# SarodYatawatta/federated-pytorch-test

Measured on NVIDIA H100. Metric: train_images_per_sec, higher is better.
Workload: dtype tf32

## Files before the change

federated_pytorch_test_b200/csrc/bindings.cpp:

```cpp
#include <ATen/cuda/CUDAContext.h>
#include <c10/cuda/CUDAGuard.h>
#include <torch/extension.h>

#include <cstdlib>

#include "fedb200.h"

namespace fb = fedb200;
using torch::Tensor;

static cudaStream_t cur_stream() { return at::cuda::getCurrentCUDAStream().stream(); }
static const float* fptr(const Tensor& t) { return t.data_ptr<float>(); }
static float* fptr_mut(Tensor& t) { return t.data_ptr<float>(); }
static const float* opt_ptr(const c10::optional<Tensor>& t) { return (t.has_value() && t->defined()) ? t->data_ptr<float>() : nullptr; }

#define CHECK_F32_CUDA(x) TORCH_CHECK((x).is_cuda() && (x).scalar_type() == torch::kFloat32, #x " must be a CUDA float32 tensor")
#define CHECK_CONTIG(x) TORCH_CHECK((x).is_contiguous(), #x " must be contiguous")

void adam_prox(Tensor x, Tensor g, Tensor m, Tensor v, Tensor step, double lr, double b1, double b2, double eps,
               c10::optional<Tensor> z, c10::optional<Tensor> y, double rho, double l1, double l2,
               c10::optional<Tensor> rho_dev) {
  CHECK_F32_CUDA(x); CHECK_CONTIG(x); CHECK_CONTIG(g); CHECK_CONTIG(m); CHECK_CONTIG(v);
  c10::cuda::CUDAGuard guard(x.device());
  fb::adam_prox(fptr_mut(x), fptr(g), fptr_mut(m), fptr_mut(v), step.data_ptr<int>(), (int)x.numel(), (float)lr, (float)b1,
// ... 262 lines not shown
  return out;
}

Tensor linear_tf32(Tensor x, Tensor w, c10::optional<Tensor> bias, bool act) {
  CHECK_F32_CUDA(x); CHECK_F32_CUDA(w); CHECK_CONTIG(x); CHECK_CONTIG(w);
  TORCH_CHECK(x.dim() == 2 && w.dim() == 2 && x.size(1) == w.size(1), "linear_tf32: x [M,K], w [N,K]");
  c10::cuda::CUDAGuard guard(x.device());
  const int M = (int)x.size(0), K = (int)x.size(1), N = (int)w.size(0);
  auto out = torch::empty({M, N}, x.options());
  fb::linear_tf32(fptr(x), fptr(w), opt_ptr(bias), fptr_mut(out), M, N, K, K, K, N, act ? 1 : 0, cur_stream());
  return out;
}
bool conv_supported(int64_t H_out, int64_t W_out, int64_t C_in, int64_t stride) {
  return fb::conv_geometry_supported((int)H_out, (int)W_out, (int)C_in, (int)stride);
}
int64_t conv_orientation(int64_t NB, int64_t H_out, int64_t W_out, int64_t C_out, int64_t stride) {
  return fb::pick_conv_orientation((int)NB, (int)H_out, (int)W_out, (int)C_out, (int)stride);
}
bool conv_window_reuse(int64_t H_out, int64_t W_out, int64_t C_in, int64_t C_out, int64_t kh, int64_t stride, int64_t dil) {
  return fb::conv_window_reuse((int)H_out, (int)W_out, (int)C_in, (int)C_out, (int)kh, (int)stride, (int)dil);
}
Tensor conv2d_nhwc(Tensor x, Tensor w, c10::optional<Tensor> stats, int64_t stride, int64_t pad, int64_t dil, int64_t orient) {
  CHECK_F32_CUDA(x); CHECK_F32_CUDA(w); CHECK_CONTIG(x); CHECK_CONTIG(w);
  TORCH_CHECK(x.dim() == 4 && w.dim() == 4 && x.size(3) == w.size(3), "conv2d_nhwc: x [N,H,W,Ci], w [Co,kh,kw,Ci]");
  c10::cuda::CUDAGuard guard(x.device());
  const int NB = (int)x.size(0), H = (int)x.size(1), W = (int)x.size(2), Ci = (int)x.size(3);
  const int Co = (int)w.size(0), kh = (int)w.size(1), kw = (int)w.size(2);
  const int Ho = (H + 2 * (int)pad - (int)dil * (kh - 1) - 1) / (int)stride + 1;
  const int Wo = (W + 2 * (int)pad - (int)dil * (kw - 1) - 1) / (int)stride + 1;
  auto y = torch::empty({NB, Ho, Wo, Co}, x.options());
  float* st = (stats.has_value() && stats->defined()) ? stats->data_ptr<float>() : nullptr;
  fb::conv2d_nhwc_tf32(fptr(x), fptr(w), fptr_mut(y), st, NB, H, W, Ci, Co, kh, kw, (int)stride, (int)pad, (int)dil, Ho, Wo, cur_stream(),
                       (int)orient);
  return y;
}

Tensor conv2d_nhwc_sized(Tensor x, Tensor w, c10::optional<Tensor> stats, int64_t stride, int64_t pad, int64_t dil,
                         int64_t Ho, int64_t Wo) {
  CHECK_F32_CUDA(x); CHECK_F32_CUDA(w); CHECK_CONTIG(x); CHECK_CONTIG(w);
  TORCH_CHECK(x.dim() == 4 && w.dim() == 4 && x.size(3) == w.size(3), "conv2d_nhwc: x [N,H,W,Ci], w [Co,kh,kw,Ci]");
  TORCH_CHECK(Ho > 0 && Wo > 0, "conv2d_nhwc_sized: positive output size");
  c10::cuda::CUDAGuard guard(x.device());
  const int NB = (int)x.size(0), H = (int)x.size(1), W = (int)x.size(2), Ci = (int)x.size(3);
  const int Co = (int)w.size(0), kh = (int)w.size(1), kw = (int)w.size(2);
  auto y = torch::empty({NB, Ho, Wo, Co}, x.options());
  float* st = (stats.has_value() && stats->defined()) ? stats->data_ptr<float>() : nullptr;
  fb::conv2d_nhwc_tf32(fptr(x), fptr(w), fptr_mut(y), st, NB, H, W, Ci, Co, kh, kw, (int)stride, (int)pad, (int)dil, (int)Ho,
                       (int)Wo, cur_stream());
  return y;
}

bool conv_wgrad_supported(int64_t Cx, int64_t Co, int64_t stride, int64_t Wo, int64_t Ho) {
  return fb::conv_wgrad_supported((int)Cx, (int)Co, (int)stride, (int)Wo, (int)Ho);
}
void conv_wgrad(Tensor x, Tensor dy, Tensor dw, int64_t stride, int64_t pad, int64_t dil) {
  CHECK_F32_CUDA(x); CHECK_F32_CUDA(dy); CHECK_F32_CUDA(dw); CHECK_CONTIG(x); CHECK_CONTIG(dy); CHECK_CONTIG(dw);
  TORCH_CHECK(x.dim() == 4 && dy.dim() == 4 && dw.dim() == 4 && x.size(0) == dy.size(0) && dw.size(0) == dy.size(3) &&
              dw.size(3) <= x.size(3), "conv_wgrad: x [N,H,W,Cx], dy [N,Ho,Wo,Co], dw [Co,kh,kw,Cw<=Cx]");
  c10::cuda::CUDAGuard guard(x.device());
  const int NB = (int)x.size(0), H = (int)x.size(1), W = (int)x.size(2), Cx = (int)x.size(3);
  const int Ho = (int)dy.size(1), Wo = (int)dy.size(2), Co = (int)dy.size(3);
  const int kh = (int)dw.size(1), kw = (int)dw.size(2), Cw = (int)dw.size(3);
  fb::conv_wgrad_tf32(fptr(x), fptr(dy), fptr_mut(dw), NB, H, W, Cx, Cw, Co, kh, kw, (int)stride, (int)pad, (int)dil, Ho, Wo,
                      cur_stream());
}

// ... 534 lines not shown
  m.def("l1_l2", &l1_l2);
  m.def("make_pair", &make_pair);
  m.def("welford", &welford);
  m.def("penalty_value", &penalty_value);
  m.def("penalty_grad", &penalty_grad);
  m.def("multi_dot", &multi_dot);
  m.def("lbfgs_two_loop", &lbfgs_two_loop);
  m.def("normalize_u8", &normalize_u8);
  m.def("augment_normalize_u8", &augment_normalize_u8, py::arg("u8"), py::arg("rows"), py::arg("key"), py::arg("counter"),
        py::arg("mean"), py::arg("std"), py::arg("to_nchw"));
  m.def("col_stats", &col_stats);
  m.def("head_fwd", &head_fwd);
  m.def("head_bwd", &head_bwd);
  m.def("bn_elu_fwd", &bn_elu_fwd, py::arg("y"), py::arg("stats"), py::arg("gamma"), py::arg("beta"), py::arg("residual"),
        py::arg("running_mean"), py::arg("running_var"), py::arg("eps"), py::arg("momentum"), py::arg("act"),
        py::arg("self_clean"), py::arg("use_running") = false);
  m.def("bn_elu_bwd", &bn_elu_bwd);
  m.def("gn_elu_fwd", &gn_elu_fwd, py::arg("y"), py::arg("gamma"), py::arg("beta"), py::arg("residual"), py::arg("groups"),
        py::arg("eps"), py::arg("act"));
  m.def("gn_elu_bwd", &gn_elu_bwd, py::arg("dout"), py::arg("out"), py::arg("y"), py::arg("mean"), py::arg("rstd"),
        py::arg("gamma"), py::arg("beta"), py::arg("groups"), py::arg("want_dres"), py::arg("act"), py::arg("want_affine"));
  m.def("avgpool_nhwc", &avgpool_nhwc);
  m.def("avgpool_nhwc_bwd", &avgpool_nhwc_bwd);
  m.def("weight_flip", &weight_flip);
  m.def("convT_pack", &convT_pack);
  m.def("linear_tf32", &linear_tf32);
  m.def("conv_supported", &conv_supported);
  m.def("conv_orientation", &conv_orientation);
  m.def("conv_window_reuse", &conv_window_reuse, py::arg("H_out"), py::arg("W_out"), py::arg("C_in"), py::arg("C_out"), py::arg("kh"),
        py::arg("stride") = 1, py::arg("dil") = 1);
  m.def("conv2d_nhwc", &conv2d_nhwc, py::arg("x"), py::arg("w"), py::arg("stats"), py::arg("stride"), py::arg("pad"), py::arg("dil"),
        py::arg("orient") = -1);
  m.def("conv2d_nhwc_sized", &conv2d_nhwc_sized);
  m.def("conv2d_nhwc_bias_act", &conv2d_nhwc_bias_act);
  m.def("conv2d_nhwc_bn_eval", &conv2d_nhwc_bn_eval);
  m.def("conv2d_nhwc_shuffle", &conv2d_nhwc_shuffle);
  m.def("conv_shuffle_supported", &conv_shuffle_supported);
  m.def("conv2d_nhwc_multidil", &conv2d_nhwc_multidil);
  m.def("conv_multidil_supported", &conv_multidil_supported);
  m.def("conv_wgrad", &conv_wgrad);
  m.def("conv_wgrad_supported", &conv_wgrad_supported);
  m.def("cross_entropy_fwd", &cross_entropy_fwd);
  m.def("cross_entropy_bwd", &cross_entropy_bwd);
  m.def("vae_loss_fwd", &vae_loss_fwd);
  m.def("vae_loss_bwd", &vae_loss_bwd);
  m.def("linear_f32", &linear_f32);
  m.def("linear_f32_dgrad", &linear_f32_dgrad);
  m.def("linear_f32_wgrad", &linear_f32_wgrad);
  m.def("act_bwd_bias", &act_bwd_bias);
  m.def("maxpool2x2_fwd", &maxpool2x2_fwd);
  m.def("maxpool2x2_bwd", &maxpool2x2_bwd);
  m.def("argmax_count", &argmax_count);
  m.def("info_nce_max_p", &info_nce_max_p);
  m.def("info_nce_scratch_floats", &info_nce_scratch_floats);
  m.def("info_nce_fwd", &info_nce_fwd);
  m.def("info_nce_bwd", &info_nce_bwd);
  m.def("gauss_nll_rows_fwd", &gauss_nll_rows_fwd);
  m.def("gauss_nll_rows_bwd", &gauss_nll_rows_bwd);
  m.def("smallconv_supported", &smallconv_supported);
  m.def("smallconv_fwd", &smallconv_fwd);
  m.def("smallconv_unpool_actbwd", &smallconv_unpool_actbwd);
  m.def("smallconv_dgrad", &smallconv_dgrad);
  m.def("smallconv_wgrad", &smallconv_wgrad);
  m.def("block_reduce", &block_reduce);
  m.def("block_reduce_fedopt", &block_reduce_fedopt);
  m.def("dp_clip", &dp_clip);
// ... 6 lines not shown
```

federated_pytorch_test_b200/csrc/fedb200.h:

```cpp
#pragma once
#include <cuda_runtime.h>
#include <stdint.h>

namespace fedb200 {

void count_launch(int n = 1);
long long launch_count();

bool pdl_enabled();
#ifdef __CUDACC__
__device__ __forceinline__ void pdl_wait() { asm volatile("griddepcontrol.wait;" ::: "memory"); }
__device__ __forceinline__ void pdl_launch_dependents() { asm volatile("griddepcontrol.launch_dependents;" ::: "memory"); }
__device__ __forceinline__ void pdl_prologue() {
  pdl_launch_dependents();
  pdl_wait();
}
template <typename... KArgs, typename... Args>
inline cudaError_t launch_pdl(void (*kernel)(KArgs...), dim3 grid, dim3 block, size_t smem, cudaStream_t stream,
                              Args&&... args) {
  cudaLaunchConfig_t cfg{};
  cfg.gridDim = grid;
  cfg.blockDim = block;
  cfg.dynamicSmemBytes = smem;
  cfg.stream = stream;
  cudaLaunchAttribute attr[1];
  attr[0].id = cudaLaunchAttributeProgrammaticStreamSerialization;
  attr[0].val.programmaticStreamSerializationAllowed = pdl_enabled() ? 1 : 0;
  cfg.attrs = attr;
  cfg.numAttrs = 1;
  return cudaLaunchKernelEx(&cfg, kernel, KArgs(args)...);
}
#endif

int pick_block_n(int M, int N);
void linear_tf32(const float* x, const float* w, const float* bias, float* out, int M, int N, int K, int ldx, int ldw,
                 int ldo, int act, cudaStream_t stream);
bool conv_geometry_supported(int H_out, int W_out, int C_in, int stride);
enum { CONV_ORIENT_AUTO = -1, CONV_ORIENT_ROW = 0, CONV_ORIENT_PIXEL = 1, CONV_ORIENT_PIXEL_PERTAP = 2 };
int pick_conv_orientation(int NB, int H_out, int W_out, int C_out, int stride);
bool conv_window_reuse(int H_out, int W_out, int C_in, int C_out, int kh, int stride, int dil);
void conv2d_nhwc_tf32(const float* x, const float* w, float* y, float* stats, int NB, int H, int W, int C_in, int C_out,
                      int kh, int kw, int stride, int pad, int dil, int H_out, int W_out, cudaStream_t stream,
                      int orient = CONV_ORIENT_AUTO);
void conv2d_nhwc_bias_act_tf32(const float* x, const float* w, const float* bias, int act, float* y, int NB, int H, int W,
                               int C_in, int C_out, int kh, int kw, int stride, int pad, int dil, int H_out, int W_out,
                               cudaStream_t stream);
void conv2d_nhwc_bn_eval_tf32(const float* x, const float* w, const float* gamma, const float* beta, const float* mean,
                              const float* var, float eps, const float* residual, int act, float* y, int NB, int H, int W,
                              int C_in, int C_out, int kh, int kw, int stride, int pad, int dil, int H_out, int W_out,
                              cudaStream_t stream);

bool conv_shuffle_supported(int H_out, int W_out, int C_in, int Ci_out);
void conv2d_nhwc_shuffle_tf32(const float* x, const float* w, float* out, int NB, int H, int W, int C_in, int C4, int kh, int kw,
                              int pad, int H_out, int W_out, cudaStream_t stream);
bool conv_multidil_supported(int H_out, int W_out, int C_in, int stride, int branches);
void conv2d_nhwc_multidil_tf32(const float* x, const float* w, const float* bias, int act, float* y, int NB, int H, int W, int C_in,
                               int C_out, int branches, int kh, int kw, int stride, const int* dils, const int* pads, int H_out,
                               int W_out, cudaStream_t stream);
bool conv_wgrad_supported(int C_x, int C_out, int stride, int W_out, int H_out);
void conv_wgrad_tf32(const float* x, const float* dy, float* dw, int NB, int H, int W, int C_x, int C_w, int C_out, int kh,
                     int kw, int stride, int pad, int dil, int H_out, int W_out, cudaStream_t stream);


void adam_prox(float* x, const float* g, float* m, float* v, const int* step_dev, int n, float lr, float b1, float b2,
               float eps, const float* z, const float* y, float rho, float l1, float l2, cudaStream_t s,
               const float* rho_dev = nullptr);
void sgd_prox(float* x, const float* g, float* buf, int n, float lr, float momentum, bool nesterov, float weight_decay,
              const float* z, const float* y, float rho, float l1, float l2, cudaStream_t s, const float* rho_dev);
void bump_step(int* step_dev, cudaStream_t s);
void l1_l2(const float* g, int n, float* out2, cudaStream_t s);
void make_pair(const float* g, const float* gprev, const float* d, float t, float trust, float* y, float* sv, int n,
               float* out3, cudaStream_t s);
void welford(const float* g, float* mean, float* m2, int n, float inv_n, float* out1, cudaStream_t s);
void penalty_value(const float* x, const float* z, const float* y, float rho, float l1, float l2, int n, float* out1,
                   cudaStream_t s);
void penalty_grad(float* g, const float* x, const float* z, const float* y, float rho, float l1, float l2, int n,
// ... 193 lines not shown
```

federated_pytorch_test_b200/csrc/gemm_wgmma.cu:

```cuda
#include "fedb200.h"
#include "igemm_wgmma.cuh"
#include "wgrad_wgmma.cuh"

#include <algorithm>
#include <cstdlib>
#include <mutex>
#include <stdexcept>
#include <string>

namespace fedb200 {

typedef CUresult (*EncodeTiledFn)(CUtensorMap*, CUtensorMapDataType, cuuint32_t, void*, const cuuint64_t*,
                                  const cuuint64_t*, const cuuint32_t*, const cuuint32_t*, CUtensorMapInterleave,
                                  CUtensorMapSwizzle, CUtensorMapL2promotion, CUtensorMapFloatOOBfill);

static EncodeTiledFn encode_fn() {
  static EncodeTiledFn fn = nullptr;
  static std::once_flag once;
  std::call_once(once, [] {
    void* p = nullptr;
    cudaDriverEntryPointQueryResult q;
    cudaError_t e = cudaGetDriverEntryPoint("cuTensorMapEncodeTiled", &p, cudaEnableDefault, &q);
    if (e != cudaSuccess || q != cudaDriverEntryPointSuccess || p == nullptr)
      throw std::runtime_error("fedb200: cuTensorMapEncodeTiled unavailable (no CUDA driver?)");
// ... 187 lines not shown

static int pix_window_stage_bytes(int H_out, int W_out, int C_in, int C_out, int kh, int stride, int dil) {
  if (C_out != 64 || stride != 1 || dil != 1 || kh != PIX_WIN_KH || C_in % IG_BLOCK_K != 0) return 0;
  if (!pix_geometry_supported(H_out, W_out, 1) || PX_BLOCK_M / W_out > H_out || (W_out * IG_BLOCK_K * 4) % 1024 != 0) return 0;
  const int win_rows = PX_BLOCK_M / W_out + kh - 1;
  if (win_rows > 256) return 0;
  const int stage = (win_rows * W_out + kh * C_out) * IG_BLOCK_K * 4;
  return PixSmem<64, PIX_WIN_STAGES>::window_total(stage) <= 227 * 1024 ? stage : 0;
}

bool conv_window_reuse(int H_out, int W_out, int C_in, int C_out, int kh, int stride, int dil) {
  return pix_window_stage_bytes(H_out, W_out, C_in, C_out, kh, stride, dil) > 0;
}

int pick_conv_orientation(int NB, int H_out, int W_out, int C_out, int stride) {
  if (env_int("FEDB200_BLOCK_N", 0) != 0) return CONV_ORIENT_ROW;
  if (C_out != 64 && C_out != 128) return CONV_ORIENT_ROW;
  if (!pix_geometry_supported(H_out, W_out, stride)) return CONV_ORIENT_ROW;
  const long long tiles = (static_cast<long long>(NB) * H_out * W_out + PX_BLOCK_M - 1) / PX_BLOCK_M;
  return tiles >= num_sms() - num_sms() / 8 ? CONV_ORIENT_PIXEL : CONV_ORIENT_ROW;
}

struct BnEvalArgs {
  const float* gamma;
  const float* beta;
  const float* mean;
  const float* var;
  float eps;
  const float* residual;
};

static void conv2d_generic(const float* x, const float* w, float* y, float* stats, const float* bias, int act, int NB, int H,
                           int W, int C_in, int C_out, int kh, int kw, int stride, int pad, int dil, int H_out, int W_out,
                           cudaStream_t stream, const BnEvalArgs* eval_bn = nullptr, int orient = CONV_ORIENT_ROW);

void conv2d_nhwc_tf32(const float* x, const float* w, float* y, float* stats, int NB, int H, int W, int C_in, int C_out,
                      int kh, int kw, int stride, int pad, int dil, int H_out, int W_out, cudaStream_t stream, int orient) {
  if (orient == CONV_ORIENT_AUTO) orient = pick_conv_orientation(NB, H_out, W_out, C_out, stride);
  conv2d_generic(x, w, y, stats, nullptr, 0, NB, H, W, C_in, C_out, kh, kw, stride, pad, dil, H_out, W_out, stream, nullptr,
                 orient);
}

void conv2d_nhwc_bias_act_tf32(const float* x, const float* w, const float* bias, int act, float* y, int NB, int H, int W,
                               int C_in, int C_out, int kh, int kw, int stride, int pad, int dil, int H_out, int W_out,
                               cudaStream_t stream) {
  conv2d_generic(x, w, y, nullptr, bias, act, NB, H, W, C_in, C_out, kh, kw, stride, pad, dil, H_out, W_out, stream);
}

void conv2d_nhwc_bn_eval_tf32(const float* x, const float* w, const float* gamma, const float* beta, const float* mean,
                              const float* var, float eps, const float* residual, int act, float* y, int NB, int H, int W,
                              int C_in, int C_out, int kh, int kw, int stride, int pad, int dil, int H_out, int W_out,
                              cudaStream_t stream) {
  const BnEvalArgs args{gamma, beta, mean, var, eps, residual};
  conv2d_generic(x, w, y, nullptr, nullptr, act, NB, H, W, C_in, C_out, kh, kw, stride, pad, dil, H_out, W_out, stream, &args);
}

static int pick_tap_pack(int C_in) {
  if (env_int("FEDB200_TAP_PACK", 1) == 0 || C_in > 16 || (C_in & 3)) return IG_BLOCK_K;
  return C_in <= 8 ? 8 : 16;
}

static void conv2d_generic(const float* x, const float* w, float* y, float* stats, const float* bias, int act, int NB, int H,
                           int W, int C_in, int C_out, int kh, int kw, int stride, int pad, int dil, int H_out, int W_out,
                           cudaStream_t stream, const BnEvalArgs* eval_bn, int orient) {
  if (!conv_geometry_supported(H_out, W_out, C_in, stride))
    throw std::runtime_error("fedb200: conv geometry not supported by the wgmma path");
  const bool pix = orient == CONV_ORIENT_PIXEL || orient == CONV_ORIENT_PIXEL_PERTAP;
  if (pix && ((C_out != 64 && C_out != 128) || bias != nullptr || act != 0 || eval_bn != nullptr ||
              !pix_geometry_supported(H_out, W_out, stride) || (reinterpret_cast<uintptr_t>(y) & 15) != 0))
    throw std::runtime_error("fedb200: pixel-major convolution needs C_out 64 / 128, a plain or statistics epilogue, "
                             "whole-row 256-pixel tiles and a 16-byte aligned output");
  const int win_stage = orient == CONV_ORIENT_PIXEL ? pix_window_stage_bytes(H_out, W_out, C_in, C_out, kh, stride, dil) : 0;
  const int tile_m = pix ? PX_BLOCK_M : IG_BLOCK_M;
  const int rows = tile_m / W_out;
  const int boxH = rows <= H_out ? rows : H_out;
  const int boxN = rows <= H_out ? 1 : rows / H_out;
  const int M = NB * H_out * W_out;
  const int bn = pix ? C_out : pick_block_n(M, C_out);
  const int cw = pick_tap_pack(C_in);
  CUtensorMap ta = make_tmap_nhwc(x, NB, H, W, C_in, boxN, win_stage ? boxH + kh - 1 : boxH, W_out, stride, cw);
  CUtensorMap tb = make_tmap_2d(w, C_out, uint64_t(kh) * kw * C_in, uint64_t(kh) * kw * C_in, bn, cw);
  IgemmParams p{};
  p.M = M; p.N = C_out;
  p.cblocks = (C_in + IG_BLOCK_K - 1) / IG_BLOCK_K;
  p.num_k_blocks = kh * kw * p.cblocks;
  p.taps_total = kh * kw;
  if (cw != IG_BLOCK_K) {
    p.cw = cw;
    p.num_k_blocks = (kh * kw + IG_BLOCK_K / cw - 1) / (IG_BLOCK_K / cw);
  }
  p.taps_w = kw; p.b_cols_per_tap = C_in; p.is_conv = 1;
  p.HW_out = H_out * W_out; p.W_out = W_out;
  p.stride = stride; p.pad = pad; p.dil = dil;
  p.out = y; p.ldo = C_out; p.bias = bias; p.act = act; p.stats = stats;
  p.k_splits = 1; p.kb_per_split = p.num_k_blocks;
  if (win_stage) {
    p.num_k_blocks = kw * p.cblocks;
    p.kb_per_split = p.num_k_blocks;
    p.win_rows = boxH + kh - 1;
    p.win_a_bytes = p.win_rows * W_out * IG_BLOCK_K * 4;
    p.win_stage_bytes = win_stage;
    launch_pix<64, PIX_WIN_KH>(ta, tb, p, stream);
    return;
  }
  if (pix) {
    if (C_out == 64) launch_pix<64, 0>(ta, tb, p, stream);
    else launch_pix<128, 0>(ta, tb, p, stream);
    return;
  }
  if (bias == nullptr && (act == 0 || eval_bn != nullptr)) {
    const int splits = pick_k_splits(M, C_out, bn, p.num_k_blocks);
    if (splits > 1) {
      p.kb_per_split = (p.num_k_blocks + splits - 1) / splits;
      p.k_splits = (p.num_k_blocks + p.kb_per_split - 1) / p.kb_per_split;
      p.stats = nullptr;
      cudaMemsetAsync(y, 0, size_t(M) * C_out * sizeof(float), stream);
    }
  }
  if (eval_bn != nullptr) {
    if ((C_out & 3) != 0) throw std::runtime_error("fedb200: eval-mode BatchNorm epilogue needs C_out % 4 == 0");
    if (p.k_splits > 1) {
      p.act = 0;
    } else {
      p.bn_gamma = eval_bn->gamma; p.bn_beta = eval_bn->beta; p.bn_mean = eval_bn->mean; p.bn_var = eval_bn->var;
      p.bn_eps = eval_bn->eps; p.residual = eval_bn->residual; p.ldr = C_out;
    }
  }
  dispatch(bn, ta, tb, p, stream);
  if (p.k_splits > 1 && stats != nullptr) col_stats(y, stats, M, C_out, stream);
  if (p.k_splits > 1 && eval_bn != nullptr)
    bn_elu_fwd(y, nullptr, eval_bn->gamma, eval_bn->beta, eval_bn->residual, y, const_cast<float*>(eval_bn->mean),
               const_cast<float*>(eval_bn->var), nullptr, nullptr, M, C_out, eval_bn->eps, 0.f, act, 0, stream, 1);
}

bool conv_shuffle_supported(int H_out, int W_out, int C_in, int Ci_out) {
  if (!conv_geometry_supported(H_out, W_out, C_in, 1)) return false;
  if (Ci_out % 32 != 0) return false;
  if (W_out > 32 || (32 % W_out) != 0) return false;
  return true;
}

void conv2d_nhwc_shuffle_tf32(const float* x, const float* w, float* out, int NB, int H, int W, int C_in, int C4, int kh, int kw,
                              int pad, int H_out, int W_out, cudaStream_t stream) {
  const int Ci = C4 / 4;
  if (!conv_shuffle_supported(H_out, W_out, C_in, Ci)) throw std::runtime_error("fedb200: shuffled conv store not supported for this shape");
  const int rows = 128 / W_out;
  const int boxH = rows <= H_out ? rows : H_out;
  const int boxN = rows <= H_out ? 1 : rows / H_out;
  const int M = NB * H_out * W_out;
// ... 134 lines not shown
```

federated_pytorch_test_b200/csrc/igemm_wgmma.cuh:

```cuda
#pragma once
#include "sm90.cuh"
#include "fedb200.h"

namespace fedb200 {

constexpr int IG_BLOCK_M = 128;
constexpr int IG_BLOCK_K = 32;
constexpr int IG_MMA_K = 8;
constexpr int IG_THREADS = 384;

struct IgemmParams {
  int M, N;
  int num_k_blocks;
  int cblocks;
  int taps_w;
  int b_cols_per_tap;
  int is_conv;
  int HW_out, W_out;
  int stride, pad, dil;
  float* out;
  int ldo;
  const float* bias;
  int act;
  float* stats;
  int kb_per_split;
  int k_splits;
  int m_tiles, n_tiles, total_tiles;
  int shuffle_ci;
  int tma_store;
  int cw;
  int taps_total;
  int ms_kh;
  unsigned long long ms_dil, ms_pad;
  const float* bn_gamma;
  const float* bn_beta;
  const float* bn_mean;
  const float* bn_var;
  float bn_eps;
  const float* residual;
  int ldr;
  int win_rows;
  int win_a_bytes;
  int win_stage_bytes;
};

template <int BLOCK_N, int STAGES>
struct IgemmSmem {
  static constexpr int A_BYTES = IG_BLOCK_M * IG_BLOCK_K * 4;
  static constexpr int B_BYTES = BLOCK_N * IG_BLOCK_K * 4;
  static constexpr int STAGE_BYTES = A_BYTES + B_BYTES;
  static constexpr int STAGING_BYTES = 2 * 64 * 32 * 4;
  static constexpr int STATS_BYTES = 8 * 2 * BLOCK_N * 4;
  static constexpr int BAR_BYTES = 2 * STAGES * 8;
  static constexpr int TOTAL = STAGES * STAGE_BYTES + STAGING_BYTES + STATS_BYTES + BAR_BYTES + 1024;
};

struct TileCoord {
  int m0, n0, kb_begin, kb_count;
};
__device__ __forceinline__ TileCoord decode_tile(const IgemmParams& p, int t, int block_m, int block_n) {
  const int n_idx = t % p.n_tiles;
  const int rest = t / p.n_tiles;
  const int m_idx = rest % p.m_tiles;
  const int z = rest / p.m_tiles;
  TileCoord c;
  c.m0 = m_idx * block_m;
  c.n0 = n_idx * block_n;
  c.kb_begin = z * p.kb_per_split;
  c.kb_count = min(p.kb_per_split, p.num_k_blocks - c.kb_begin);
  return c;
}

__device__ __forceinline__ void named_bar_sync(uint32_t id, uint32_t n) {
  asm volatile("bar.sync %0, %1;" ::"r"(id), "r"(n) : "memory");
}
__device__ __forceinline__ void named_bar_arrive(uint32_t id, uint32_t n) {
// ... 212 lines not shown
          }
        }
      }
    }
    if (p.tma_store) {
#pragma unroll
      for (int c0 = 0; c0 < BLOCK_N; c0 += 32) {
        if (tid == 0) tma_store_wait_read();
        named_bar_sync(wg_bar, 128);
#pragma unroll
        for (int ii = 0; ii < 4; ++ii) {
          const int i = c0 / 8 + ii;
          const int cc = 8 * ii + col_in;
#pragma unroll
          for (int h = 0; h < 2; ++h) {
            const int r = row_in + 8 * h;
            const int rr = r & 31;
            float* dst = stg + (r >> 5) * 1024 + rr * 32 + (((uint32_t(cc) >> 2) ^ uint32_t(rr & 7)) << 2) + (cc & 3);
            *reinterpret_cast<float2*>(dst) = make_float2(acc[4 * i + 2 * h], acc[4 * i + 2 * h + 1]);
          }
        }
        fence_proxy_async();
        named_bar_sync(wg_bar, 128);
        if (tid == 0) {
          const int pc = c.n0 + c0;
          for (int b = 0; b < 2; ++b) {
            const int row0 = c.m0 + 64 * g + 32 * b;
            if (row0 >= p.M || pc >= p.N) continue;
            const float* src = stg + b * 1024;
            if (p.shuffle_ci > 0) {
              const int phase = pc / p.shuffle_ci;
              if (p.k_splits > 1) tma_reduce_add_5d(&tmap_c, src, pc - phase * p.shuffle_ci, phase & 1, 0, phase >> 1, row0 / p.W_out);
              else tma_store_5d(&tmap_c, src, pc - phase * p.shuffle_ci, phase & 1, 0, phase >> 1, row0 / p.W_out);
            } else if (p.k_splits > 1) {
              tma_reduce_add_2d(&tmap_c, src, pc, row0);
            } else {
              tma_store_2d(&tmap_c, src, pc, row0);
            }
          }
          tma_store_commit();
        }
      }
    } else {
#pragma unroll
      for (int i = 0; i < NACC / 4; ++i) {
#pragma unroll
        for (int h = 0; h < 2; ++h) {
          const int row = h ? row_b : row_a;
          if (!(h ? ok_b : ok_a)) continue;
#pragma unroll
          for (int e = 0; e < 2; ++e) {
            const int col = c.n0 + 8 * i + col_in + e;
            if (col >= p.N) continue;
            float* dst = p.out + size_t(row) * p.ldo + col;
            if (p.k_splits > 1) atomicAdd(dst, acc[4 * i + 2 * h + e]);
            else *dst = acc[4 * i + 2 * h + e];
          }
        }
      }
    }
    if (p.stats != nullptr) {
      named_bar_sync(3, 256);
      for (int j = threadIdx.x - 128; j < 2 * BLOCK_N; j += 256) {
        float v = 0.f;
#pragma unroll
        for (int w = 0; w < 8; ++w) v += colsum[w * 2 * BLOCK_N + j];
        const int cc = j < BLOCK_N ? j : j - BLOCK_N;
        if (c.n0 + cc < p.N) atomicAdd(p.stats + (j < BLOCK_N ? 0 : p.N) + c.n0 + cc, v);
      }
      named_bar_sync(3, 256);
    }
  }
  if (p.tma_store && tid == 0) tma_store_wait_read();
}

constexpr int PX_BLOCK_M = 256;

template <int CO, int STAGES>
struct PixSmem {
  static constexpr int A_BYTES = PX_BLOCK_M * IG_BLOCK_K * 4;
  static constexpr int B_BYTES = CO * IG_BLOCK_K * 4;
  static constexpr int STAGE_BYTES = A_BYTES + B_BYTES;
  static constexpr int STAGING_BYTES = 2 * 2 * 2 * 32 * 32 * 4;
  static constexpr int BAR_BYTES = 2 * STAGES * 8;
  static constexpr int TOTAL = STAGES * STAGE_BYTES + STAGING_BYTES + BAR_BYTES + 1024;
  static constexpr int window_total(int stage_bytes) { return STAGES * stage_bytes + STAGING_BYTES + BAR_BYTES + 1024; }
};

// ... 158 lines not shown
      if ((lane & 3) == 0) {
        const int ca = ch_wg + ch_lo;
        atomicAdd(p.stats + ca, s1a);
        atomicAdd(p.stats + p.N + ca, s2a);
        atomicAdd(p.stats + ca + 8, s1b);
        atomicAdd(p.stats + p.N + ca + 8, s2b);
      }
    }
#pragma unroll
    for (int q = 0; q < PX_BLOCK_M / 32; ++q) {
      float* buf = stg + (q & 1) * 2048;
      if (tid == 0) tma_store_wait_read_n<1>();
      named_bar_sync(wg_bar, 128);
#pragma unroll
      for (int ii = 0; ii < 4; ++ii) {
        const int i = 4 * q + ii;
#pragma unroll
        for (int h = 0; h < 2; ++h) {
          const int ch = ch_lo + 8 * h;
          const int cc = ch & 31;
#pragma unroll
          for (int e = 0; e < 2; ++e) {
            const int px = 8 * ii + px_in + e;
            buf[(ch >> 5) * 1024 + px * 32 + (((uint32_t(cc) >> 2) ^ uint32_t(px & 7)) << 2) + (cc & 3)] = acc[4 * i + 2 * h + e];
          }
        }
      }
      fence_proxy_async();
      named_bar_sync(wg_bar, 128);
      if (tid == 0) {
        const int row0 = c.m0 + 32 * q;
        if (row0 < p.M) {
#pragma unroll
          for (int b = 0; b < 2; ++b) tma_store_2d(&tmap_c, buf + b * 1024, ch_wg + 32 * b, row0);
        }
        tma_store_commit();
      }
    }
  }
  if (tid == 0) tma_store_wait_read();
}

}
```

federated_pytorch_test_b200/models/resnet.py:

```python
from __future__ import annotations

import functools
from typing import Callable, List, Type

import torch
import torch.nn as nn
import torch.nn.functional as F

from .base import BlockPartitioned
from ..ops import functional as FX


def _conv3x3(cin: int, cout: int, stride: int) -> nn.Conv2d:
    return nn.Conv2d(cin, cout, kernel_size=3, stride=stride, padding=1, bias=False)


def _conv1x1(cin: int, cout: int, stride: int) -> nn.Conv2d:
    return nn.Conv2d(cin, cout, kernel_size=1, stride=stride, bias=False)


def norm_layer(norm: str = "batch", groups: int = 32) -> Callable[[int], nn.Module]:
    if norm == "batch":
        return nn.BatchNorm2d
    if norm == "group":
        return functools.partial(nn.GroupNorm, groups)
    raise ValueError("norm must be 'batch' or 'group', got %r" % (norm,))


class _Residual(nn.Module):

    expansion = 1

    def _make_shortcut(self, in_planes: int, out_planes: int, stride: int, norm) -> None:
        if stride != 1 or in_planes != out_planes:
            self.shortcut = nn.Sequential(_conv1x1(in_planes, out_planes, stride), norm(out_planes))
        else:
            self.shortcut = nn.Sequential()

    def _skip(self, x: torch.Tensor) -> torch.Tensor:
        if len(self.shortcut) == 0:
            return x
        return FX.conv_bn_act(x, self.shortcut[0], self.shortcut[1], act=False)


class BasicBlock(_Residual):
    expansion = 1

    def __init__(self, in_planes: int, planes: int, stride: int = 1, norm=nn.BatchNorm2d):
        super().__init__()
        self.conv1 = _conv3x3(in_planes, planes, stride)
        self.bn1 = norm(planes)
        self.conv2 = _conv3x3(planes, planes, 1)
        self.bn2 = norm(planes)
        self._make_shortcut(in_planes, planes * self.expansion, stride, norm)

    def forward(self, x: torch.Tensor) -> torch.Tensor:
        h = FX.conv_bn_act(x, self.conv1, self.bn1, act=True)
        return FX.conv_bn_act(h, self.conv2, self.bn2, residual=self._skip(x), act=True)


class Bottleneck(_Residual):
    expansion = 4

    def __init__(self, in_planes: int, planes: int, stride: int = 1, norm=nn.BatchNorm2d):
        super().__init__()
        self.conv1 = _conv1x1(in_planes, planes, 1)
        self.bn1 = norm(planes)
        self.conv2 = _conv3x3(planes, planes, stride)
        self.bn2 = norm(planes)
        self.conv3 = _conv1x1(planes, planes * self.expansion, 1)
        self.bn3 = norm(planes * self.expansion)
        self._make_shortcut(in_planes, planes * self.expansion, stride, norm)

    def forward(self, x: torch.Tensor) -> torch.Tensor:
        h = FX.conv_bn_act(x, self.conv1, self.bn1, act=True)
        h = FX.conv_bn_act(h, self.conv2, self.bn2, act=True)
        return FX.conv_bn_act(h, self.conv3, self.bn3, residual=self._skip(x), act=True)


class ResNet(BlockPartitioned):
    _TABLES = {
        18: ((0, 2), (3, 8), (9, 14), (15, 23), (24, 29), (30, 38), (39, 44), (45, 53), (54, 59), (60, 61)),
        9: ((0, 2), (3, 8), (9, 14), (15, 17), (18, 23), (24, 29), (30, 32), (33, 37)),
    }
    LINEAR_IDS = ()

    def __init__(self, block: Type[_Residual], num_blocks: List[int], qualifier: int, num_classes: int = 10,
                 norm: str = "batch", groups: int = 32):
        super().__init__()
# ... 36 lines not shown
```

federated_pytorch_test_b200/ops/cuda_ops.py:

```python
from __future__ import annotations

from typing import List, Optional, Sequence, Tuple

import torch
import torch.nn as nn
import torch.nn.functional as F

from .. import _ext
from . import conv_math

_EXT = None


def ext():
    global _EXT
    if _EXT is None:
        _EXT = _ext.load("fedb200_cuda", required=True)
    return _EXT


def launch_count() -> int:
    return int(ext().launch_count())


# ... 305 lines not shown
    def forward(ctx, x, weight, gamma, beta, residual, running_mean, running_var, stride, pad, eps, momentum, act):
        e = ext()
        xn = _nhwc(x)
        wk = _krsc(weight)
        if xn.shape[3] == 3:
            xn = F.pad(xn, (0, 1))
            wk = F.pad(wk, (0, 1))
        Co = weight.shape[0]
        stats, self_clean = _stats_buffer(weight, Co)
        y = e.conv2d_nhwc(xn, wk, stats, stride, pad, 1)
        res = _nhwc(residual) if residual is not None else None
        out, mean, invstd = e.bn_elu_fwd(y, stats, gamma, beta, res, running_mean, running_var, eps, momentum, act, self_clean)
        ctx.save_for_backward(xn, wk, y, out, mean, invstd, gamma, beta)
        ctx.cfg = (stride, pad, act, residual is not None, tuple(weight.shape), x.shape[1])
        ctx.w_persistent = _aliases(wk, weight)
        ctx.weight_ref = weight
        return out.permute(0, 3, 1, 2)

    @staticmethod
    def backward(ctx, dout):
        e = ext()
        xn, wk, y, out, mean, invstd, gamma, beta = ctx.saved_tensors
        stride, pad, act, has_res, wshape, cin_logical = ctx.cfg
        need_x, need_w, need_g, need_b, need_r = ctx.needs_input_grad[:5]
        dn = _nhwc(dout)
        dgamma = torch.zeros_like(gamma) if need_g else None
        dbeta = torch.zeros_like(gamma) if need_b else None
        dy, dres = e.bn_elu_bwd(dn, out if (has_res or not act) else None, y, mean, invstd, gamma, beta, dgamma, dbeta,
                                bool(has_res and need_r), act, _bwd_sums_buffer(gamma, gamma.numel()))
        dx, dw = _conv_backward(e, xn, wk, dy, stride, pad, wshape, cin_logical, need_x, need_w, ctx.w_persistent,
                                ctx.weight_ref)
        dr = dres.permute(0, 3, 1, 2) if (has_res and need_r and dres is not None) else None
        return dx, dw, dgamma, dbeta, dr, None, None, None, None, None, None, None


def _conv_backward(e, xn, wk, dy, stride, pad, wshape, cin_logical, need_x, need_w, w_persistent, weight_ref):
    dx = dw = None
    kh, kw = wshape[2], wshape[3]
    if need_x:
        Ci = xn.shape[3]
        if stride == 1 and e.conv_supported(xn.shape[1], xn.shape[2], wshape[0], 1) and Ci % 4 == 0:
            dxn = e.conv2d_nhwc(dy, _flipped_weight(wk, need_w, w_persistent), None, 1, kh - 1 - pad, 1)
        elif stride == 2 and _s2_dgrad_supported(e, xn, dy, kh, kw, pad):
            dxn = _s2_dgrad(e, dy, wk, need_w, w_persistent)
        else:
            dxn = torch.ops.aten.convolution_backward(
                dy.permute(0, 3, 1, 2), xn.permute(0, 3, 1, 2), wk.permute(0, 3, 1, 2), None,
                [stride, stride], [pad, pad], [1, 1], False, [0, 0], 1, [True, False, False])[0]
            dxn = _nhwc(dxn)
        if dxn.shape[3] != cin_logical:
            dxn = dxn[..., :cin_logical]
        dx = dxn.permute(0, 3, 1, 2)
    if need_w:
        if conv_wgrad_supported(xn, dy, stride):
            dw = conv_wgrad(xn, dy, kh, kw, cin_logical, stride, pad, 1, weight_ref)
        else:
            dwk = torch.ops.aten.convolution_backward(
                dy.permute(0, 3, 1, 2), xn.permute(0, 3, 1, 2), wk.permute(0, 3, 1, 2), None,
                [stride, stride], [pad, pad], [1, 1], False, [0, 0], 1, [False, True, False])[1]
            dw = dwk[:, :cin_logical] if dwk.shape[1] != cin_logical else dwk
    return dx, dw


def conv_gn_act_supported(x: torch.Tensor, conv: nn.Conv2d, gn: nn.GroupNorm) -> bool:
    if not isinstance(gn, nn.GroupNorm) or not gn.affine or gn.weight.dtype != torch.float32:
        return False
# ... 585 lines not shown
```

federated_pytorch_test_b200/ops/functional.py:

```python
from __future__ import annotations

import os
from typing import Optional

import torch
import torch.nn as nn
import torch.nn.functional as F

_FAST = {"enabled": os.environ.get("FEDB200_FAST", "1") != "0"}


def set_fast_path(flag: bool) -> None:
    _FAST["enabled"] = bool(flag)


def fast_path_enabled() -> bool:
    return _FAST["enabled"]


def _use_fast(x: torch.Tensor) -> bool:
    return _FAST["enabled"] and x.is_cuda


def conv_bn_act(
    x: torch.Tensor,
    conv: nn.Conv2d,
    bn: nn.BatchNorm2d,
    residual: Optional[torch.Tensor] = None,
    act: bool = True,
) -> torch.Tensor:
    if _use_fast(x):
        from . import cuda_ops

        if cuda_ops.conv_bn_act_eval_supported(x, conv, bn, residual):
            return cuda_ops.conv_bn_act_eval(x, conv, bn, residual, act)
        if cuda_ops.conv_bn_act_supported(x, conv, bn):
            return cuda_ops.conv_bn_act(x, conv, bn, residual, act)
        if cuda_ops.conv_gn_act_supported(x, conv, bn):
            return cuda_ops.conv_gn_act(x, conv, bn, residual, act)
    y = F.conv2d(x, conv.weight, conv.bias, conv.stride, conv.padding, conv.dilation, conv.groups)
    y = bn(y)
    if residual is not None:
        y = y + residual
    return F.elu(y) if act else y


def pool_linear(x: torch.Tensor, linear: nn.Linear, window: int = 4) -> torch.Tensor:
    if _use_fast(x):
        from . import cuda_ops

        if cuda_ops.pool_linear_supported(x, linear, window):
            return cuda_ops.pool_linear(x, linear, window)
    y = F.avg_pool2d(x, window)
    return F.linear(y.reshape(y.shape[0], -1), linear.weight, linear.bias)


def conv_act(x: torch.Tensor, conv: nn.Module, act: bool = True) -> torch.Tensor:
    if _use_fast(x):
        from . import cuda_ops

        if cuda_ops.conv_act_supported(x, conv) or cuda_ops.conv_transpose_act_supported(x, conv):
            return cuda_ops.conv_act(x, conv, act)
        if cuda_ops.conv1x1_supported(x, conv):
            return cuda_ops.conv1x1_linear(x, conv, act)
        if cuda_ops.unfold_conv_supported(x, conv):
            return cuda_ops.unfold_conv(x, conv, act)
        if cuda_ops.smallconv_supported(x, conv):
            return cuda_ops.small_conv(x, conv, act, False)
    y = conv(x)
    return F.elu(y) if act else y


def dilated_stem(x: torch.Tensor, convs, act: bool = True) -> torch.Tensor:
    if _use_fast(x):
        from . import cuda_ops

        if cuda_ops.dilated_stem_supported(x, convs):
# ... 43 lines not shown
```

Measured before the change: 36590.

## Fuse residual skip gradient into conv data-gradient via accumulating store

```diff
diff --git a/baseline/profile_step.py b/baseline/profile_step.py
--- /dev/null
+++ b/baseline/profile_step.py
@@ -0,0 +1,124 @@
+from __future__ import annotations
+
+import argparse
+import collections
+import json
+import os
+import subprocess
+import sys
+
+import torch
+
+ROOT = os.path.dirname(os.path.dirname(os.path.abspath(__file__)))
+if ROOT not in sys.path:
+    sys.path.insert(0, ROOT)
+
+STEPS_PER_ROUND = 49
+CATEGORIES = ("conv forward", "data gradient", "weight gradient", "bn_elu_fwd", "bn_elu_bwd reduce/apply",
+              "ATen elementwise", "head / loss / optimizer", "rest")
+
+
+def category(name: str, backward: bool) -> str:
+    if "igemm_wgmma" in name:
+        return "data gradient" if backward else "conv forward"
+    if "wgrad_wgmma" in name:
+        return "weight gradient"
+    if "bn_elu_fwd" in name:
+        return "bn_elu_fwd"
+    if "bn_elu_bwd" in name:
+        return "bn_elu_bwd reduce/apply"
+    if "at::native" in name or "elementwise" in name.lower():
+        return "ATen elementwise"
+    if any(k in name for k in ("head_", "ce_fwd", "ce_bwd", "adam_prox", "sgd_prox", "bump_step", "avgpool", "penalty")):
+        return "head / loss / optimizer"
+    return "rest"
+
+
+def device_info() -> str:
+    try:
+        q = subprocess.run(["nvidia-smi", "--query-gpu=name,power.limit,clocks.max.sm", "--format=csv,noheader"],
+                           capture_output=True, text=True, timeout=30).stdout.strip()
+    except (OSError, subprocess.SubprocessError):
+        q = ""
+    return q or torch.cuda.get_device_name()
+
+
+def main() -> None:
+    ap = argparse.ArgumentParser()
+    ap.add_argument("--warmup", type=int, default=8)
+    ap.add_argument("--steps", type=int, default=20)
+    args = ap.parse_args()
+    assert torch.cuda.is_available(), "profile_step.py measures on the GPU"
+    assert args.warmup + 2 * args.steps < STEPS_PER_ROUND, "both windows must lie inside the first round"
+
+    from federated_pytorch_test_b200.algo.engine import Engine
+    from federated_pytorch_test_b200.algo.strategies import FedAvg
+    from federated_pytorch_test_b200.api import common, federated_multi
+
+    cfg = federated_multi.Config(K=1, use_resnet=True, Nloop=1000, Nadmm=3, Nepoch=1, check_results=False, save_model=False,
+                                 be_verbose=False, biased_input=True, data_on_device=True, graphs=True, fast=True,
+                                 collective="auto", diagnostics="post", max_minibatches=STEPS_PER_ROUND, seed=69,
+                                 optimizer="adam")
+    topo, coll = common.setup_runtime(cfg)
+    task = common.ClassifierTask(cfg, topo, cfg.lambda1, cfg.lambda2)
+    eng = Engine(task, topo, FedAvg(coll, topo), coll, common.engine_config(cfg), log=lambda m: None)
+
+    p0, p1 = args.warmup, args.warmup + args.steps
+    t1 = p1 + args.steps
+    prof = torch.profiler.profile(activities=[torch.profiler.ProfilerActivity.CUDA])
+    ev = [torch.cuda.Event(enable_timing=True), torch.cuda.Event(enable_timing=True)]
+
+    def hook(e: Engine) -> None:
+        n = e.steps_done
+        if n == p0:
+            torch.cuda.synchronize()
+            prof.start()
+        elif n == p1:
+            torch.cuda.synchronize()
+            prof.stop()
+            ev[0].record()
+        elif n == t1:
+            ev[1].record()
+            torch.cuda.synchronize()
+            e.stop_requested = True
+
+    eng.step_hook = hook
+    eng.run()
+    step_ms = ev[0].elapsed_time(ev[1]) / args.steps
+
+    kernels = sorted((k for k in prof.events() if k.device_type == torch.autograd.DeviceType.CUDA and k.device_time > 0),
+                     key=lambda k: k.time_range.start)
+    per_name = collections.defaultdict(float)
+    launches = collections.Counter()
+    backward = False
+    for k in kernels:
+        name = k.name
+        if "ce_bwd" in name or "head_bwd" in name:
+            backward = True
+        cat = category(name, backward)
+        if "adam_prox" in name or "sgd_prox" in name:
+            backward = False
+        short = name.split("(")[0].replace("void ", "").replace("fedb200::", "")
+        per_name[(cat, short)] += k.device_time / 1e3 / args.steps
+        launches[(cat, short)] += 1
+    per_cat = collections.defaultdict(float)
+    for (cat, _), t in per_name.items():
+        per_cat[cat] += t
+    total = sum(per_cat.values())
+
+    print("device:", device_info())
+    print("%-28s %10s %8s" % ("category / kernel", "us/step", "launches"))
+    for cat in CATEGORIES:
+        print("%-28s %10.1f" % (cat, per_cat.get(cat, 0.0) * 1e3))
+        for (c, short), t in sorted(per_name.items(), key=lambda kv: -kv[1]):
+            if c == cat:
+                print("    %-50s %8.1f %6.1f" % (short[:50], t * 1e3, launches[(c, short)] / args.steps))
+    print("kernel sum %.1f us/step, event-timed step %.1f us, between kernels %.1f us"
+          % (total * 1e3, step_ms * 1e3, (step_ms - total) * 1e3))
+    print(json.dumps({"device": device_info(), "step_ms": round(step_ms, 4), "kernel_sum_ms": round(total, 4),
+                      "categories_us": {c: round(per_cat.get(c, 0.0) * 1e3, 1) for c in CATEGORIES},
+                      "launches_per_step": {"%s|%s" % k: v / args.steps for k, v in sorted(launches.items())}}))
+
+
+if __name__ == "__main__":
+    main()
diff --git a/federated_pytorch_test_b200/csrc/bindings.cpp b/federated_pytorch_test_b200/csrc/bindings.cpp
--- a/federated_pytorch_test_b200/csrc/bindings.cpp
+++ b/federated_pytorch_test_b200/csrc/bindings.cpp
@@ -318,6 +318,21 @@
   float* st = (stats.has_value() && stats->defined()) ? stats->data_ptr<float>() : nullptr;
   fb::conv2d_nhwc_tf32(fptr(x), fptr(w), fptr_mut(y), st, NB, H, W, Ci, Co, kh, kw, (int)stride, (int)pad, (int)dil, Ho, Wo, cur_stream(),
                        (int)orient);
+  return y;
+}
+
+Tensor conv2d_nhwc_accumulate(Tensor x, Tensor w, Tensor y, int64_t stride, int64_t pad, int64_t dil) {
+  CHECK_F32_CUDA(x); CHECK_F32_CUDA(w); CHECK_F32_CUDA(y); CHECK_CONTIG(x); CHECK_CONTIG(w); CHECK_CONTIG(y);
+  TORCH_CHECK(x.dim() == 4 && w.dim() == 4 && y.dim() == 4 && x.size(3) == w.size(3),
+              "conv2d_nhwc_accumulate: x [N,H,W,Ci], w [Co,kh,kw,Ci]");
+  c10::cuda::CUDAGuard guard(x.device());
+  const int NB = (int)x.size(0), H = (int)x.size(1), W = (int)x.size(2), Ci = (int)x.size(3);
+  const int Co = (int)w.size(0), kh = (int)w.size(1), kw = (int)w.size(2);
+  const int Ho = (H + 2 * (int)pad - (int)dil * (kh - 1) - 1) / (int)stride + 1;
+  const int Wo = (W + 2 * (int)pad - (int)dil * (kw - 1) - 1) / (int)stride + 1;
+  TORCH_CHECK(y.size(0) == NB && y.size(1) == Ho && y.size(2) == Wo && y.size(3) == Co, "conv2d_nhwc_accumulate: y must be [N,Ho,Wo,Co]");
+  fb::conv2d_nhwc_accumulate_tf32(fptr(x), fptr(w), fptr_mut(y), NB, H, W, Ci, Co, kh, kw, (int)stride, (int)pad, (int)dil, Ho, Wo,
+                                  cur_stream());
   return y;
 }
 
@@ -918,6 +933,7 @@
   m.def("conv2d_nhwc", &conv2d_nhwc, py::arg("x"), py::arg("w"), py::arg("stats"), py::arg("stride"), py::arg("pad"), py::arg("dil"),
         py::arg("orient") = -1);
   m.def("conv2d_nhwc_sized", &conv2d_nhwc_sized);
+  m.def("conv2d_nhwc_accumulate", &conv2d_nhwc_accumulate);
   m.def("conv2d_nhwc_bias_act", &conv2d_nhwc_bias_act);
   m.def("conv2d_nhwc_bn_eval", &conv2d_nhwc_bn_eval);
   m.def("conv2d_nhwc_shuffle", &conv2d_nhwc_shuffle);
diff --git a/federated_pytorch_test_b200/csrc/fedb200.h b/federated_pytorch_test_b200/csrc/fedb200.h
--- a/federated_pytorch_test_b200/csrc/fedb200.h
+++ b/federated_pytorch_test_b200/csrc/fedb200.h
@@ -42,6 +42,8 @@
 void conv2d_nhwc_tf32(const float* x, const float* w, float* y, float* stats, int NB, int H, int W, int C_in, int C_out,
                       int kh, int kw, int stride, int pad, int dil, int H_out, int W_out, cudaStream_t stream,
                       int orient = CONV_ORIENT_AUTO);
+void conv2d_nhwc_accumulate_tf32(const float* x, const float* w, float* y, int NB, int H, int W, int C_in, int C_out, int kh,
+                                 int kw, int stride, int pad, int dil, int H_out, int W_out, cudaStream_t stream);
 void conv2d_nhwc_bias_act_tf32(const float* x, const float* w, const float* bias, int act, float* y, int NB, int H, int W,
                                int C_in, int C_out, int kh, int kw, int stride, int pad, int dil, int H_out, int W_out,
                                cudaStream_t stream);
diff --git a/federated_pytorch_test_b200/csrc/gemm_wgmma.cu b/federated_pytorch_test_b200/csrc/gemm_wgmma.cu
--- a/federated_pytorch_test_b200/csrc/gemm_wgmma.cu
+++ b/federated_pytorch_test_b200/csrc/gemm_wgmma.cu
@@ -243,13 +243,21 @@
 
 static void conv2d_generic(const float* x, const float* w, float* y, float* stats, const float* bias, int act, int NB, int H,
                            int W, int C_in, int C_out, int kh, int kw, int stride, int pad, int dil, int H_out, int W_out,
-                           cudaStream_t stream, const BnEvalArgs* eval_bn = nullptr, int orient = CONV_ORIENT_ROW);
+                           cudaStream_t stream, const BnEvalArgs* eval_bn = nullptr, int orient = CONV_ORIENT_ROW,
+                           int accumulate = 0);
 
 void conv2d_nhwc_tf32(const float* x, const float* w, float* y, float* stats, int NB, int H, int W, int C_in, int C_out,
                       int kh, int kw, int stride, int pad, int dil, int H_out, int W_out, cudaStream_t stream, int orient) {
   if (orient == CONV_ORIENT_AUTO) orient = pick_conv_orientation(NB, H_out, W_out, C_out, stride);
   conv2d_generic(x, w, y, stats, nullptr, 0, NB, H, W, C_in, C_out, kh, kw, stride, pad, dil, H_out, W_out, stream, nullptr,
                  orient);
+}
+
+void conv2d_nhwc_accumulate_tf32(const float* x, const float* w, float* y, int NB, int H, int W, int C_in, int C_out, int kh,
+                                 int kw, int stride, int pad, int dil, int H_out, int W_out, cudaStream_t stream) {
+  const int orient = pick_conv_orientation(NB, H_out, W_out, C_out, stride);
+  conv2d_generic(x, w, y, nullptr, nullptr, 0, NB, H, W, C_in, C_out, kh, kw, stride, pad, dil, H_out, W_out, stream, nullptr,
+                 orient, 1);
 }
 
 void conv2d_nhwc_bias_act_tf32(const float* x, const float* w, const float* bias, int act, float* y, int NB, int H, int W,
@@ -273,7 +281,7 @@
 
 static void conv2d_generic(const float* x, const float* w, float* y, float* stats, const float* bias, int act, int NB, int H,
                            int W, int C_in, int C_out, int kh, int kw, int stride, int pad, int dil, int H_out, int W_out,
-                           cudaStream_t stream, const BnEvalArgs* eval_bn, int orient) {
+                           cudaStream_t stream, const BnEvalArgs* eval_bn, int orient, int accumulate) {
   if (!conv_geometry_supported(H_out, W_out, C_in, stride))
     throw std::runtime_error("fedb200: conv geometry not supported by the wgmma path");
   const bool pix = orient == CONV_ORIENT_PIXEL || orient == CONV_ORIENT_PIXEL_PERTAP;
@@ -305,6 +313,7 @@
   p.stride = stride; p.pad = pad; p.dil = dil;
   p.out = y; p.ldo = C_out; p.bias = bias; p.act = act; p.stats = stats;
   p.k_splits = 1; p.kb_per_split = p.num_k_blocks;
+  p.accumulate = accumulate;
   if (win_stage) {
     p.num_k_blocks = kw * p.cblocks;
     p.kb_per_split = p.num_k_blocks;
@@ -325,7 +334,7 @@
       p.kb_per_split = (p.num_k_blocks + splits - 1) / splits;
       p.k_splits = (p.num_k_blocks + p.kb_per_split - 1) / p.kb_per_split;
       p.stats = nullptr;
-      cudaMemsetAsync(y, 0, size_t(M) * C_out * sizeof(float), stream);
+      if (!accumulate) cudaMemsetAsync(y, 0, size_t(M) * C_out * sizeof(float), stream);
     }
   }
   if (eval_bn != nullptr) {
diff --git a/federated_pytorch_test_b200/csrc/igemm_wgmma.cuh b/federated_pytorch_test_b200/csrc/igemm_wgmma.cuh
--- a/federated_pytorch_test_b200/csrc/igemm_wgmma.cuh
+++ b/federated_pytorch_test_b200/csrc/igemm_wgmma.cuh
@@ -42,6 +42,7 @@
   int win_rows;
   int win_a_bytes;
   int win_stage_bytes;
+  int accumulate;
 };
 
 template <int BLOCK_N, int STAGES>
@@ -320,7 +321,7 @@
               const int phase = pc / p.shuffle_ci;
               if (p.k_splits > 1) tma_reduce_add_5d(&tmap_c, src, pc - phase * p.shuffle_ci, phase & 1, 0, phase >> 1, row0 / p.W_out);
               else tma_store_5d(&tmap_c, src, pc - phase * p.shuffle_ci, phase & 1, 0, phase >> 1, row0 / p.W_out);
-            } else if (p.k_splits > 1) {
+            } else if (p.k_splits > 1 || p.accumulate) {
               tma_reduce_add_2d(&tmap_c, src, pc, row0);
             } else {
               tma_store_2d(&tmap_c, src, pc, row0);
@@ -341,7 +342,7 @@
             const int col = c.n0 + 8 * i + col_in + e;
             if (col >= p.N) continue;
             float* dst = p.out + size_t(row) * p.ldo + col;
-            if (p.k_splits > 1) atomicAdd(dst, acc[4 * i + 2 * h + e]);
+            if (p.k_splits > 1 || p.accumulate) atomicAdd(dst, acc[4 * i + 2 * h + e]);
             else *dst = acc[4 * i + 2 * h + e];
           }
         }
@@ -566,7 +567,10 @@
         const int row0 = c.m0 + 32 * q;
         if (row0 < p.M) {
 #pragma unroll
-          for (int b = 0; b < 2; ++b) tma_store_2d(&tmap_c, buf + b * 1024, ch_wg + 32 * b, row0);
+          for (int b = 0; b < 2; ++b) {
+            if (p.accumulate) tma_reduce_add_2d(&tmap_c, buf + b * 1024, ch_wg + 32 * b, row0);
+            else tma_store_2d(&tmap_c, buf + b * 1024, ch_wg + 32 * b, row0);
+          }
         }
         tma_store_commit();
       }
diff --git a/federated_pytorch_test_b200/models/resnet.py b/federated_pytorch_test_b200/models/resnet.py
--- a/federated_pytorch_test_b200/models/resnet.py
+++ b/federated_pytorch_test_b200/models/resnet.py
@@ -55,6 +55,9 @@
         self._make_shortcut(in_planes, planes * self.expansion, stride, norm)
 
     def forward(self, x: torch.Tensor) -> torch.Tensor:
+        if len(self.shortcut) == 0:
+            h, skip = FX.conv_bn_act_skip(x, self.conv1, self.bn1)
+            return FX.conv_bn_act(h, self.conv2, self.bn2, residual=skip, act=True)
         h = FX.conv_bn_act(x, self.conv1, self.bn1, act=True)
         return FX.conv_bn_act(h, self.conv2, self.bn2, residual=self._skip(x), act=True)
 
diff --git a/federated_pytorch_test_b200/ops/cuda_ops.py b/federated_pytorch_test_b200/ops/cuda_ops.py
--- a/federated_pytorch_test_b200/ops/cuda_ops.py
+++ b/federated_pytorch_test_b200/ops/cuda_ops.py
@@ -361,6 +361,56 @@
                                 ctx.weight_ref)
         dr = dres.permute(0, 3, 1, 2) if (has_res and need_r and dres is not None) else None
         return dx, dw, dgamma, dbeta, dr, None, None, None, None, None, None, None
+
+
+def conv_bn_act_skip_supported(x: torch.Tensor, conv: nn.Conv2d, bn: nn.BatchNorm2d) -> bool:
+    if not conv_bn_act_supported(x, conv, bn) or x.shape[1] % 4:
+        return False
+    kh, kw = conv.kernel_size
+    if conv.stride != (1, 1) or kh != kw or 2 * conv.padding[0] != kh - 1 or conv.out_channels != x.shape[1]:
+        return False
+    return bool(ext().conv_supported(x.shape[2], x.shape[3], conv.out_channels, 1))
+
+
+class _ConvBnActSkip(torch.autograd.Function):
+
+    @staticmethod
+    def forward(ctx, x, weight, gamma, beta, running_mean, running_var, pad, eps, momentum):
+        e = ext()
+        xn = _nhwc(x)
+        wk = _krsc(weight)
+        stats, self_clean = _stats_buffer(weight, weight.shape[0])
+        y = e.conv2d_nhwc(xn, wk, stats, 1, pad, 1)
+        out, mean, invstd = e.bn_elu_fwd(y, stats, gamma, beta, None, running_mean, running_var, eps, momentum, True, self_clean)
+        ctx.save_for_backward(xn, wk, y, mean, invstd, gamma, beta)
+        ctx.cfg = (pad, tuple(weight.shape))
+        ctx.w_persistent = _aliases(wk, weight)
+        ctx.weight_ref = weight
+        return out.permute(0, 3, 1, 2), x.view_as(x)
+
+    @staticmethod
+    def backward(ctx, dout, dskip):
+        e = ext()
+        xn, wk, y, mean, invstd, gamma, beta = ctx.saved_tensors
+        pad, wshape = ctx.cfg
+        need_x, need_w, need_g, need_b = ctx.needs_input_grad[:4]
+        dgamma = torch.zeros_like(gamma) if need_g else None
+        dbeta = torch.zeros_like(gamma) if need_b else None
+        dy, _ = e.bn_elu_bwd(_nhwc(dout), None, y, mean, invstd, gamma, beta, dgamma, dbeta, False, True,
+                             _bwd_sums_buffer(gamma, gamma.numel()))
+        fuse = need_x and dskip is not None
+        dx, dw = _conv_backward(e, xn, wk, dy, 1, pad, wshape, wshape[1], need_x and not fuse, need_w, ctx.w_persistent,
+                                ctx.weight_ref)
+        if fuse:
+            acc = _nhwc(dskip)
+            e.conv2d_nhwc_accumulate(dy, _flipped_weight(wk, need_w, ctx.w_persistent), acc, 1, wshape[2] - 1 - pad, 1)
+            dx = acc.permute(0, 3, 1, 2)
+        return dx, dw, dgamma, dbeta, None, None, None, None, None
+
+
+def conv_bn_act_skip(x, conv: nn.Conv2d, bn: nn.BatchNorm2d):
+    return _ConvBnActSkip.apply(x, conv.weight, bn.weight, bn.bias, bn.running_mean, bn.running_var, conv.padding[0], bn.eps,
+                                bn.momentum)
 
 
 def _conv_backward(e, xn, wk, dy, stride, pad, wshape, cin_logical, need_x, need_w, w_persistent, weight_ref):
diff --git a/federated_pytorch_test_b200/ops/functional.py b/federated_pytorch_test_b200/ops/functional.py
--- a/federated_pytorch_test_b200/ops/functional.py
+++ b/federated_pytorch_test_b200/ops/functional.py
@@ -43,6 +43,15 @@
     if residual is not None:
         y = y + residual
     return F.elu(y) if act else y
+
+
+def conv_bn_act_skip(x: torch.Tensor, conv: nn.Conv2d, bn: nn.BatchNorm2d):
+    if _use_fast(x):
+        from . import cuda_ops
+
+        if cuda_ops.conv_bn_act_skip_supported(x, conv, bn):
+            return cuda_ops.conv_bn_act_skip(x, conv, bn)
+    return conv_bn_act(x, conv, bn, act=True), x
 
 
 def pool_linear(x: torch.Tensor, linear: nn.Linear, window: int = 4) -> torch.Tensor:
```

Measured after the change: 37310 (median of 6 runs). +1.9%, better.
